# aerius-labs/indexed-merkle-tree-halo2

Measured on AMD Instinct MI355X. Metric: indexed-tree insertions/sec at depth=32 (bn256::Fr), higher is better.
Workload: dtype u32 limbs (9 x 29-bit, Montgomery mod p), 64-bit accumulate

## Files before the change

### indexed-merkle-tree-halo2_amd/csrc/imt_capi.cpp

```cpp
#include "imt_ctx.hpp"
#include "imt_gadget.hpp"
#include <cstring>
#include <new>

using namespace imt;

void* imt_ctx::dev_scratch(size_t slot, size_t bytes) {
    if (slot >= scratch.size()) scratch.resize(slot + 1);
    Scratch& s = scratch[slot];
    if (s.cap >= bytes && s.p) return s.p;
    if (s.p) {
        hipStreamSynchronize(stream);
        hipFree(s.p);
        s.p = nullptr;
        s.cap = 0;
    }
    size_t cap = bytes < 4096 ? 4096 : bytes + bytes / 4;
    hipError_t e = hipMalloc(&s.p, cap);
    if (e != hipSuccess) {
        s.p = nullptr;
        hip_fail(e, "hipMalloc(scratch)");
        return nullptr;
    }
    s.cap = cap;
// ... 105 lines not shown
    IMT_HIP(c, hipStreamSynchronize(c->stream));
    for (auto st : c->side_streams) IMT_HIP(c, hipStreamSynchronize(st));
    for (auto& p : c->prof_pending) {
        float ms = 0;
        if (hipEventElapsedTime(&ms, p.a, p.b) == hipSuccess) {
            c->prof_ms[p.cls] += ms;
            c->prof_n[p.cls] += 1;
        }
        c->prof_pool.push_back(p.a);
        c->prof_pool.push_back(p.b);
    }
    c->prof_pending.clear();
    for (int k = 0; k < IMT_PROF_ALL_CLASSES; k++) {
        if (k < classes) {
            out[2 * k] = c->prof_ms[k];
            out[2 * k + 1] = c->prof_n[k];
        }
        c->prof_ms[k] = c->prof_n[k] = 0;
    }
    return IMT_OK;
}
extern "C" int imt_profile_read(imt_ctx* c, double* out) { return profile_read(c, out, IMT_PROF_CLASSES); }
extern "C" int imt_profile_read_all(imt_ctx* c, double* out) { return profile_read(c, out, IMT_PROF_ALL_CLASSES); }

extern "C" int imt_ctx_set_option(imt_ctx* c, int option, uint64_t value) {
    if (!c) return IMT_ERR_ARG;
    switch (option) {
        case IMT_OPT_COOP_MAX_EVENTS:
            if (value > 0xffffffffu) return c->fail(IMT_ERR_RANGE, "value out of range");
            c->coop_max_events = (uint32_t)value;
            return IMT_OK;
        default:
            return c->fail(IMT_ERR_ARG, "unknown option %d", option);
    }
}

extern "C" const char* imt_version(void) { return "imt-hip gfx950 r4"; }

extern "C" int imt_ctx_create(int device, imt_ctx** out) {
    if (!out) return IMT_ERR_ARG;
    *out = nullptr;
    if (device < 0) return IMT_ERR_NO_DEVICE;
    int count = 0;
    if (hipGetDeviceCount(&count) != hipSuccess || count <= 0 || device >= count) return IMT_ERR_NO_DEVICE;
    imt_ctx* c = new (std::nothrow) imt_ctx();
    if (!c) return IMT_ERR_ALLOC;
    c->device = device;
    std::string err;
    if (!c->hp.init(err)) { delete c; return IMT_ERR_INTERNAL; }
    dev::PoseidonConsts pc;
    c->hp.fill_consts(pc);
    dev::TraceConsts tc;
    c->hp.fill_trace_consts(tc);
    hipError_t e;
    if ((e = hipSetDevice(device)) != hipSuccess || (e = hipStreamCreate(&c->own_stream)) != hipSuccess ||
        (e = launch::upload_consts(pc)) != hipSuccess || (e = launch::upload_trace_consts(tc)) != hipSuccess || (e = hipMalloc((void**)&c->d_err, sizeof(int))) != hipSuccess ||
        (e = hipMalloc((void**)&c->d_zero, (IMT_MAX_DEPTH + 1) * 32)) != hipSuccess) {
        if (c->own_stream) hipStreamDestroy(c->own_stream);
        if (c->d_err) hipFree(c->d_err);
        delete c;
        return e == hipErrorNoDevice ? IMT_ERR_NO_DEVICE : IMT_ERR_HIP;
    }
    c->stream = c->own_stream;
    e = hipMemsetAsync(c->d_err, 0, sizeof(int), c->stream);
    launch::zero_chain(c->stream, c->d_zero, IMT_MAX_DEPTH);
    if (e != hipSuccess || (e = hipStreamSynchronize(c->stream)) != hipSuccess) {
        imt_ctx_destroy(c);
        return IMT_ERR_HIP;
    }
    *out = c;
    return IMT_OK;
}

extern "C" void imt_ctx_destroy(imt_ctx* c) {
    if (!c) return;
    hipSetDevice(c->device);
    hipStreamSynchronize(c->stream);
    for (auto& s : c->scratch)
        if (s.p) hipFree(s.p);
    for (auto& p : c->prof_pending) { hipEventDestroy(p.a); hipEventDestroy(p.b); }
    for (auto& e : c->prof_pool) hipEventDestroy(e);
    if (c->d_err) hipFree(c->d_err);
    if (c->d_zero) hipFree(c->d_zero);
    if (c->own_stream) hipStreamDestroy(c->own_stream);
    delete c;
}

extern "C" const char* imt_last_error(const imt_ctx* c) { return c ? c->last_error.c_str() : "null context"; }

extern "C" int imt_ctx_set_stream(imt_ctx* c, void* s) {
    if (!c) return IMT_ERR_ARG;
    c->stream = s ? (hipStream_t)s : c->own_stream;
    return IMT_OK;
}

extern "C" int imt_ctx_sync(imt_ctx* c) {
    if (!c) return IMT_ERR_ARG;
    int rc = c->set_device();
    if (rc) return rc;
    for (auto st : c->side_streams) IMT_HIP(c, hipStreamSynchronize(st));
    return c->sync_and_check();
}

namespace {

struct Io {
    imt_ctx* c;
    unsigned flags;
    bool dev;
// ... 666 lines not shown
```

### indexed-merkle-tree-halo2_amd/csrc/imt_consts.hpp

```cpp
#pragma once
#include <cstdint>

namespace imt {
namespace dev {

constexpr int NL = 9;
constexpr uint32_t MASK29 = (1u << 29) - 1;

struct Fe {
    uint32_t v[NL];
};

constexpr int RF = 8, RP = 57;
struct PoseidonConsts {
    Fe rc_full[RF][3];
    Fe rc_h2p2[3];
    Fe k_partial[RP];
    Fe mats[2][3][3];
    Fe sp_row[RP][3];
    Fe sp_col[RP][2];
    Fe cap0;
    Fe one;
    Fe from_canon;
    Fe from_mont256;
    Fe to_mont256;
    Fe int_one;
    Fe zero_leaf;
    Fe sc_rc[RF][3];
    Fe sc_mats[RF][3][3];
    Fe rec_k[RP];
    Fe rec_c[RP][4];
    Fe rec_exit[2][3];
    Fe rec_unused[51];
};

struct TraceConsts {
    Fe absorb[3][3];
    Fe full_c[RF][3];
    Fe partial[RP];
    Fe mats[2][3][3];
    Fe row[RP][3];
    Fe col_hat[RP][2];
};
constexpr int TRACE_ROWS_H2 = 1208, TRACE_ROWS_H3 = 1209;

}
}
```

### indexed-merkle-tree-halo2_amd/csrc/imt_kernels.hip

```cpp
#include <algorithm>
#include <hip/hip_runtime.h>
#include <hip/hip_ext.h>

#include "imt_device.hpp"
#include "imt_trace_device.hpp"
#include "imt_launch.hpp"
#include "imt_sweep.hpp"
#if defined(__HIP_DEVICE_COMPILE__)
#include "imt_coop_device.hpp"
#endif

namespace imt {

__constant__ dev::PoseidonConsts g_pc;
__constant__ dev::TraceConsts g_tc;

namespace {
using namespace dev;

#ifndef IMT_BLOCK
#define IMT_BLOCK 256
#endif
#ifndef IMT_HASH_WAVES
#define IMT_HASH_WAVES __attribute__((amdgpu_waves_per_eu(5, 5)))
#endif
#ifndef IMT_COOP_WAVES
#define IMT_COOP_WAVES __attribute__((amdgpu_waves_per_eu(1, 2)))
#endif
constexpr int BLOCK = IMT_BLOCK;

__device__ __forceinline__ size_t gtid() { return (size_t)blockIdx.x * blockDim.x + threadIdx.x; }
__device__ __forceinline__ size_t gtid_again() {
    uint32_t lo = blockIdx.x * blockDim.x + threadIdx.x, hi = (uint32_t)(((uint64_t)blockIdx.x * blockDim.x + threadIdx.x) >> 32);
    asm volatile("" : "+v"(lo), "+v"(hi));
    return ((size_t)hi << 32) | lo;
}
__device__ __forceinline__ void flag_err(int* err, bool ok) {
    if (!ok && err) atomicOr(err, 1);
}

__device__ __forceinline__ void to_int(Fe& r, const Fe& a) {
    mont_mul(r, a, g_pc.int_one);
    canonicalize(r);
}
__device__ __forceinline__ bool int_lt(const Fe& a, const Fe& b) {
    bool lt = false;
#pragma unroll
    for (int i = 0; i < NL; i++) {
        if (a.v[i] != b.v[i]) lt = a.v[i] < b.v[i];
    }
    return lt;
}
__device__ __forceinline__ void fe_from_u64(Fe& r, uint64_t x) {
    Fe t;
#pragma unroll
    for (int i = 0; i < NL; i++) t.v[i] = 0;
    t.v[0] = (uint32_t)x & MASK29;
    t.v[1] = (uint32_t)(x >> 29) & MASK29;
    t.v[2] = (uint32_t)(x >> 58);
    mont_mul(r, t, g_pc.from_canon);
    canonicalize(r);
}

__device__ __forceinline__ void order_pair(Fe& A, Fe& B, bool right, const Fe& cur, const Fe& sv) {
#pragma unroll
    for (int i = 0; i < NL; i++) {
        A.v[i] = right ? sv.v[i] : cur.v[i];
// ... 644 lines not shown
}

struct StoredSibling {
    __device__ __forceinline__ const uint8_t* operator()(const launch::SweepArgs& a, int32_t ss, uint64_t sn) const {
        return ss >= 0 ? a.val_in + (size_t)ss * 32 : (sn < a.len_l ? a.tree_l + sn * 32 : a.zero_l);
    }
};
struct ViewSibling {
    const view::Side& side;
    __device__ __forceinline__ const uint8_t* operator()(const launch::SweepArgs& a, int32_t ss, uint64_t sn) const {
        return replay::sibling_row(side, ss, a.level, sn, a.val_in, a.tree_l, a.len_l, a.zero_l);
    }
};
#if defined(__HIP_DEVICE_COMPILE__)
template <bool TABLES, class Sibling, class Rows = InsertRows>
__device__ __forceinline__ void sweep_body_quad(const launch::SweepArgs& a, Sibling sibling, uint32_t* tab, Rows rows = Rows()) {
    coop::tab_fill(tab, g_pc);
    const size_t t = gtid();
    const size_t q = t >> 2;
    if (q >= a.count) return;
    const unsigned role = (unsigned)t & 3u, ri = role == 3u ? 0u : role;
    const uint32_t x = a.begin + (uint32_t)q;
    const bool leaves = !TABLES && a.mode == launch::SWEEP_LEAVES;
    Fe X, C3, o;
    C3 = g_pc.one;
    if (leaves) {
        flag_err(a.err, leaf_inputs_quad(X, C3, a.pre + (size_t)a.time0[x] * 96, a.fmt_in, ri));
    } else {
        uint32_t k = x, n = 0, e = x;
        const uint8_t* sp = a.zero_l;
        if (TABLES || a.from) {
            k = a.from[x] & ~sweep::LAST_BIT;
            n = a.node_below[x];
            e = a.time_next[x];
            sp = sibling(a, a.sibsrc[x], (uint64_t)(n ^ 1u));
        }
        Fe cur, sv;
        load_packed(cur, a.val_in + (size_t)k * 32);
        load_packed(sv, sp);
        pick_input(X, ri, n & 1u, cur, sv);
        if (role == 0u) {
            if (!TABLES && x == a.last_event && a.node_in) store_packed(a.node_in, cur);
            rows(a, e, sv);
        }
    }
    coop::hash23(tab, o, X, C3, leaves, ri);
    if (role == 1u) {
        store_packed(a.val_out + (size_t)x * 32, o);
        if (!TABLES && x == a.last_event && a.node_out) store_packed(a.node_out, o);
    }
}
#endif
__global__ IMT_HASH_WAVES void __launch_bounds__(BLOCK) k_sweep(launch::SweepArgs a) {
    __shared__ uint32_t stash[NL][BLOCK];
    const size_t t = gtid();
    if (t >= a.count) return;
    const uint32_t x = a.begin + (uint32_t)t;
    Fe A, B, o;
    if (a.mode == launch::SWEEP_LEAVES) {
        const uint8_t* p = a.pre + (size_t)a.time0[x] * 96;
        Fe C;
        bool ok = load_fe(g_pc, A, p, a.fmt_in);
        ok &= load_fe(g_pc, B, p + 32, a.fmt_in);
        ok &= load_fe(g_pc, C, p + 64, a.fmt_in);
#pragma unroll
        for (int i = 0; i < NL; i++) stash[i][threadIdx.x] = C.v[i];
        flag_err(a.err, ok);
    } else {
        uint32_t k = x, n = 0, e = x;
        const uint8_t* sp = a.zero_l;
        if (a.from) {
            k = a.from[x] & ~sweep::LAST_BIT;
            n = a.node_below[x];
            e = a.time_next[x];
            const int32_t ss = a.sibsrc[x];
            const uint64_t sn = (uint64_t)(n ^ 1u);
            sp = ss >= 0 ? a.val_in + (size_t)ss * 32 : (sn < a.len_l ? a.tree_l + sn * 32 : a.zero_l);
        }
        Fe cur, sv;
        load_packed(cur, a.val_in + (size_t)k * 32);
        load_packed(sv, sp);
        if (x == a.last_event && a.node_in) store_packed(a.node_in, cur);
        const bool right = n & 1u;
#pragma unroll
        for (int i = 0; i < NL; i++) {
            A.v[i] = right ? sv.v[i] : cur.v[i];
            B.v[i] = right ? cur.v[i] : sv.v[i];
        }
        uint8_t* row = (e & 1u) ? a.new_sib : a.low_sib;
        if (row) store_fe(g_pc, row + ((uint64_t)a.level * a.lay.level_stride + (uint64_t)(e >> 1) * a.lay.item_stride) * 32, sv, a.fmt_out);
    }
    hash23_stashed(g_pc, o, A, B, a.mode == launch::SWEEP_LEAVES, &stash[0][threadIdx.x], BLOCK);
    store_packed(a.val_out + (size_t)x * 32, o);
    if (x == a.last_event && a.node_out) store_packed(a.node_out, o);
}

__global__ IMT_HASH_WAVES void __launch_bounds__(BLOCK) k_sweep_coop(launch::SweepArgs a) {
#if defined(__HIP_DEVICE_COMPILE__)
    __shared__ uint32_t tab[coop::TAB_DWORDS];
    sweep_body_quad<false>(a, StoredSibling(), tab);
#endif
}

__global__ IMT_HASH_WAVES void __launch_bounds__(BLOCK) k_sweep_mixed(launch::SweepMixedArgs m) {
    const launch::SweepArgs& a = m.sweep;
    const size_t t = gtid();
    if (t >= a.count) return;
    const uint32_t x = a.begin + (uint32_t)t;
    uint32_t k = x, n = 0, e = x;
    const uint8_t* sp = a.zero_l;
    if (a.from) {
        k = a.from[x] & ~sweep::LAST_BIT;
        n = a.node_below[x];
        e = a.time_next[x];
        sp = StoredSibling()(a, a.sibsrc[x], (uint64_t)(n ^ 1u));
    }
    Fe A, B, o, cur, sv;
    load_packed(cur, a.val_in + (size_t)k * 32);
    load_packed(sv, sp);
    if (x == a.last_event && a.node_in) store_packed(a.node_in, cur);
    order_pair(A, B, n & 1u, cur, sv);
    MixedRows{m.erow, m.read_sib}(a, e, sv);
    hash23_stashed(g_pc, o, A, B, false, nullptr, 0);
    store_packed(a.val_out + (size_t)x * 32, o);
    if (x == a.last_event && a.node_out) store_packed(a.node_out, o);
}

__global__ IMT_HASH_WAVES void __launch_bounds__(BLOCK) k_sweep_mixed_coop(launch::SweepMixedArgs m) {
#if defined(__HIP_DEVICE_COMPILE__)
    __shared__ uint32_t tab[coop::TAB_DWORDS];
    sweep_body_quad<false>(m.sweep, StoredSibling(), tab, MixedRows{m.erow, m.read_sib});
#endif
}

__global__ void __launch_bounds__(BLOCK)
k_emit_roots_mixed(const uint8_t* __restrict__ val, uint32_t total, const uint32_t* __restrict__ erow, uint32_t n_ins,
                   uint8_t* __restrict__ old_root, uint8_t* __restrict__ interim_root, uint8_t* __restrict__ new_root,
                   uint8_t* __restrict__ read_root, unsigned fmt_out, uint8_t* __restrict__ node_store) {
    const size_t t = gtid();
    if (t >= total) return;
    const uint32_t e = (uint32_t)t;
    Fe cur;
    load_packed(cur, val + (size_t)e * 32);
    if (e == total - 1 && node_store) store_packed(node_store, cur);
    const uint32_t w = erow[e], kind = w & 3u;
    const size_t i = w >> 2;
    if (kind == 1u) {
// ... 440 lines not shown
        const uint32_t* nodes = reinterpret_cast<const uint32_t*>(j.payload + 128 + (size_t)j.cap * 32);
        const uint64_t node = nodes[i];
        if (node >= j.len_l) return;
        const Word4* s = reinterpret_cast<const Word4*>(j.payload + 128 + i * 32);
        Word4* d = reinterpret_cast<Word4*>(j.tree_l + node * 32);
        d[0] = s[0];
        d[1] = s[1];
        return;
    }
    if (i >= 3) return;
    uint8_t* dst = i == 0 ? j.node_in : (i == 1 ? j.node_out : j.root);
    if (!dst) return;
    const Word4* s = reinterpret_cast<const Word4*>(j.payload + i * 32);
    Word4* d = reinterpret_cast<Word4*>(dst);
    d[0] = s[0];
    d[1] = s[1];
}

__global__ void k_store_top_path(const uint8_t* __restrict__ top_path, uint8_t* __restrict__ tree_nodes,
                                 const uint64_t* __restrict__ tree_off, unsigned l0, unsigned depth) {
    const unsigned l = l0 + threadIdx.x;
    if (l > depth) return;
    const Word4* s = reinterpret_cast<const Word4*>(top_path + (size_t)(l - l0) * 32);
    Word4* d = reinterpret_cast<Word4*>(tree_nodes + tree_off[l] * 32);
    d[0] = s[0];
    d[1] = s[1];
}

__global__ void __launch_bounds__(256) k_mad_peak(uint32_t* out, uint32_t seed, int iters) {
    uint64_t a0 = threadIdx.x + seed, a1 = a0 * 3 + 1, a2 = a0 * 5 + 2, a3 = a0 * 7 + 3;
    uint64_t a4 = a0 * 11 + 4, a5 = a0 * 13 + 5, a6 = a0 * 17 + 6, a7 = a0 * 19 + 7;
    const uint32_t b = (uint32_t)a0 | 1u, c = seed * 77u + 12345u;
    for (int i = 0; i < iters; i++) {
        asm volatile("v_mad_u64_u32 %0, vcc, %8, %9, %0\n v_mad_u64_u32 %1, vcc, %8, %9, %1\n"
                     "v_mad_u64_u32 %2, vcc, %8, %9, %2\n v_mad_u64_u32 %3, vcc, %8, %9, %3\n"
                     "v_mad_u64_u32 %4, vcc, %8, %9, %4\n v_mad_u64_u32 %5, vcc, %8, %9, %5\n"
                     "v_mad_u64_u32 %6, vcc, %8, %9, %6\n v_mad_u64_u32 %7, vcc, %8, %9, %7\n"
                     : "+v"(a0), "+v"(a1), "+v"(a2), "+v"(a3), "+v"(a4), "+v"(a5), "+v"(a6), "+v"(a7)
                     : "v"(b), "v"(c) : "vcc");
    }
    const uint64_t r = a0 ^ a1 ^ a2 ^ a3 ^ a4 ^ a5 ^ a6 ^ a7;
    out[blockIdx.x * blockDim.x + threadIdx.x] = (uint32_t)r ^ (uint32_t)(r >> 32);
}

inline unsigned nblk(size_t n) { return (unsigned)((n + BLOCK - 1) / BLOCK); }

}

namespace launch {

hipError_t upload_consts(const dev::PoseidonConsts& pc) {
    return hipMemcpyToSymbol(HIP_SYMBOL(g_pc), &pc, sizeof(pc), 0, hipMemcpyHostToDevice);
}
hipError_t upload_trace_consts(const dev::TraceConsts& tc) {
    return hipMemcpyToSymbol(HIP_SYMBOL(g_tc), &tc, sizeof(tc), 0, hipMemcpyHostToDevice);
}
void hash_trace_jobs(hipStream_t s, const TraceJobs& a, unsigned fmt_out) {
    size_t most = 0;
    for (int k = 0; k < a.n_jobs; k++) most = std::max(most, a.j[k].n_items);
    if (!most || a.n_jobs <= 0) return;
    auto* k = fmt_out == FMT_MONT256 ? k_hash_trace<FMT_MONT256>
              : fmt_out == FMT_DEVICE ? k_hash_trace<FMT_DEVICE> : k_hash_trace<FMT_CANONICAL>;
    hipLaunchKernelGGL(k, dim3(nblk(most), (unsigned)a.n_jobs), dim3(BLOCK), 0, s, a);
}
void hash_trace(hipStream_t s, const uint8_t* in, size_t n_items, int arity, uint8_t* trace, size_t n_per, size_t row0,
                size_t rows_total, bool item_major, unsigned fmt_in, unsigned fmt_out, int* err) {
    TraceJobs a{};
    a.j[0] = {in, n_items, arity, row0, fmt_in};
    a.n_jobs = 1;
    a.trace = trace; a.n_per = n_per; a.rows_total = rows_total; a.item_major = item_major ? 1 : 0; a.err = err;
    hash_trace_jobs(s, a, fmt_out);
}
void insert_trace_inputs(hipStream_t s, const uint8_t* low_leaf, const uint8_t* new_leaf, const uint64_t* new_index,
                         size_t n, uint8_t* new_low, uint8_t* zero_leaf, unsigned fmt, int* err) {
    if (!n) return;
    hipLaunchKernelGGL(k_insert_trace_inputs, dim3(nblk(n)), dim3(BLOCK), 0, s, low_leaf, new_leaf, new_index, n, new_low,
                       zero_leaf, fmt, err);
}
void path_pairs(hipStream_t s, const PathChains& a, uint32_t coop_max) {
    if (!a.n || a.n_chains <= 0) return;
    if (a.n * 4 * (size_t)a.n_chains <= coop_max)
        hipLaunchKernelGGL(k_path_pairs_coop, dim3(nblk(a.n * 4), (unsigned)a.n_chains), dim3(BLOCK), 0, s, a);
    else
        hipLaunchKernelGGL(k_path_pairs, dim3(nblk(a.n), (unsigned)a.n_chains), dim3(BLOCK), 0, s, a);
}

void hash_batch(hipStream_t s, const uint8_t* in, uint8_t* out, size_t n, int arity, unsigned fmt_in,
                unsigned fmt_out, int* err, uint32_t coop_max) {
    if (!n) return;
    if (n * 4 <= coop_max)
        hipLaunchKernelGGL(k_hash_batch_coop, dim3(nblk(n * 4)), dim3(BLOCK), 0, s, in, out, n, arity, fmt_in, fmt_out, err);
    else
        hipLaunchKernelGGL(k_hash_batch, dim3(nblk(n)), dim3(BLOCK), 0, s, in, out, n, arity, fmt_in, fmt_out, err);
}
void permute_batch(hipStream_t s, const uint8_t* in, uint8_t* out, size_t n, unsigned fmt_in, unsigned fmt_out,
                   int* err) {
    if (!n) return;
    hipLaunchKernelGGL(k_permute_batch, dim3(nblk(n)), dim3(BLOCK), 0, s, in, out, n, fmt_in, fmt_out, err);
}
void convert(hipStream_t s, const uint8_t* in, uint8_t* out, size_t n, unsigned fmt_in, unsigned fmt_out,
             int* err) {
    if (!n) return;
    hipLaunchKernelGGL(k_convert, dim3(nblk(n)), dim3(BLOCK), 0, s, in, out, n, fmt_in, fmt_out, err);
}
void split128(hipStream_t s, const uint8_t* vals, uint8_t* q, uint8_t* r, size_t n, unsigned fmt, int* err) {
    if (!n) return;
// ... 33 lines not shown
                    unsigned fmt_in, unsigned fmt_out, int* err, uint32_t coop_max) {
    (void)fmt_out;
    if (!n) return;
    if (n * 16 <= coop_max)
        hipLaunchKernelGGL(k_insert_chains_coop, dim3(nblk(n * 4), 4), dim3(BLOCK), 0, s, low_leaf, low_index, low_sib,
                           new_leaf, new_index, new_path_index, new_sib, lay, depth, n, trace, fmt_in, err);
    else
        hipLaunchKernelGGL(k_insert_chains, dim3(nblk(n), 4), dim3(BLOCK), 0, s, low_leaf, low_index, low_sib, new_leaf,
                           new_index, new_path_index, new_sib, lay, depth, n, trace, fmt_in, err);
    hipLaunchKernelGGL(k_insert_check, dim3(nblk(n)), dim3(BLOCK), 0, s, old_root, low_leaf, new_root, new_leaf,
                       is_largest, n, trace, fail_out, fmt_in, err);
}
void tree_level(hipStream_t s, const uint8_t* prev, uint8_t* next, size_t n_parents, uint32_t coop_max) {
    if (!n_parents) return;
    if (n_parents * 4 <= coop_max)
        hipLaunchKernelGGL(k_hash_batch_coop, dim3(nblk(n_parents * 4)), dim3(BLOCK), 0, s, prev, next, n_parents, 2,
                           (unsigned)FMT_DEVICE, (unsigned)FMT_DEVICE, (int*)nullptr);
    else
        hipLaunchKernelGGL(k_tree_level, dim3(nblk(n_parents)), dim3(BLOCK), 0, s, prev, next, n_parents);
}
void index_leaves(hipStream_t s, const uint8_t* val, const uint32_t* sorted, uint32_t M, uint64_t base, uint8_t* tree0,
                  int* err) {
    if (!M) return;
    hipLaunchKernelGGL(k_index_leaves, dim3(nblk(M)), dim3(BLOCK), 0, s, val, sorted, M, base, tree0, err);
}
void zero_chain(hipStream_t s, uint8_t* out, unsigned depth) {
    hipLaunchKernelGGL(k_zero_chain, dim3(1), dim3(64), 0, s, out, depth);
}
void extend_root(hipStream_t s, uint8_t* cur, const uint8_t* zero, unsigned from, unsigned to) {
    hipLaunchKernelGGL(k_extend_root, dim3(1), dim3(64), 0, s, cur, zero, from, to);
}
void gather_proof(hipStream_t s, TreeView tv, const uint64_t* index, size_t n, unsigned depth, uint8_t* out,
                  SibLayout lay, unsigned fmt_out) {
    if (!n || !depth) return;
    hipLaunchKernelGGL(k_gather_proof, dim3(nblk(n * depth)), dim3(BLOCK), 0, s, tv, index, n, depth, out, lay,
                       fmt_out);
}
void write_helpers(hipStream_t s, uint64_t index, unsigned depth, uint8_t* out, unsigned fmt_out) {
    if (!depth) return;
    hipLaunchKernelGGL(k_write_helpers, dim3((depth + 63) / 64), dim3(64), 0, s, index, depth, out, fmt_out);
}


void mad_peak(hipStream_t s, uint32_t* out, unsigned blocks, int iters) {
    hipLaunchKernelGGL(k_mad_peak, dim3(blocks), dim3(256), 0, s, out, 1u, iters);
}
void fill_level(hipStream_t s, uint8_t* nodes, size_t n, const uint8_t* zero_l) {
    if (!n) return;
    hipLaunchKernelGGL(k_fill_level, dim3(nblk(n)), dim3(BLOCK), 0, s, nodes, n, zero_l);
}
static void launch_sweep(hipStream_t s, const SweepArgs& a, uint32_t coop_max) {
    if (a.count <= coop_max)
        hipLaunchKernelGGL(k_sweep_coop, dim3(nblk((size_t)a.count * 4)), dim3(BLOCK), 0, s, a);
    else
        hipLaunchKernelGGL(k_sweep, dim3(nblk(a.count)), dim3(BLOCK), 0, s, a);
}
void sweep_leaves(hipStream_t s, const uint8_t* pre, const uint32_t* time0, uint8_t* val0, uint32_t k_begin,
                  uint32_t k_count, unsigned fmt_in, int* err, uint32_t coop_max) {
    if (!k_count) return;
    SweepArgs a{};
    a.mode = SWEEP_LEAVES;
    a.begin = k_begin; a.count = k_count;
    a.pre = pre; a.time0 = time0; a.val_out = val0; a.fmt_in = fmt_in; a.err = err;
    a.last_event = 0xffffffffu;
    launch_sweep(s, a, coop_max);
}
void merge_level(hipStream_t s, sweep::LevelTable in, sweep::LevelOut out, uint32_t total) {
    if (!total) return;
    hipLaunchKernelGGL(k_merge_level, dim3(nblk(total)), dim3(BLOCK), 0, s, in, out, total);
}
static SweepArgs level_args(const uint8_t* val_in, uint8_t* val_out, const uint32_t* from, const int32_t* sibsrc,
                            const uint32_t* node_below, const uint32_t* time_next, const uint8_t* tree_l, uint64_t len_l,
                            const uint8_t* zero_l, uint32_t k_begin, uint32_t k_count, uint8_t* low_sib, uint8_t* new_sib,
                            SibLayout lay, unsigned level, unsigned fmt_out) {
    SweepArgs a{};
    a.mode = SWEEP_LEVEL;
    a.begin = k_begin; a.count = k_count;
    a.val_in = val_in; a.val_out = val_out; a.from = from; a.sibsrc = sibsrc; a.node_below = node_below;
    a.time_next = time_next; a.tree_l = tree_l; a.len_l = len_l; a.zero_l = zero_l; a.level = level;
    a.low_sib = low_sib; a.new_sib = new_sib; a.lay = lay; a.fmt_out = fmt_out;
    a.last_event = 0xffffffffu;
    return a;
}
void sweep_level(hipStream_t s, const uint8_t* val_in, uint8_t* val_out, const uint32_t* from, const int32_t* sibsrc,
                 const uint32_t* node_below, const uint32_t* time_next, const uint8_t* tree_l, uint64_t len_l,
                 const uint8_t* zero_l, uint32_t k_begin, uint32_t k_count, uint8_t* low_sib, uint8_t* new_sib,
                 SibLayout lay, unsigned level, unsigned fmt_out, uint32_t coop_max) {
    if (!k_count) return;
    launch_sweep(s, level_args(val_in, val_out, from, sibsrc, node_below, time_next, tree_l, len_l, zero_l, k_begin, k_count,
                               low_sib, new_sib, lay, level, fmt_out), coop_max);
}
void sweep_upper(hipStream_t s, const uint8_t* val_in, uint8_t* val_out, const uint8_t* zero_l, uint32_t e_begin,
                 uint32_t e_count, uint32_t last_event, uint8_t* node_in, uint8_t* node_out, uint8_t* low_sib,
                 uint8_t* new_sib, SibLayout lay, unsigned level, unsigned fmt_out, uint32_t coop_max) {
    if (!e_count) return;
    SweepArgs a{};
    a.mode = SWEEP_LEVEL;
    a.begin = e_begin; a.count = e_count;
    a.val_in = val_in; a.val_out = val_out; a.zero_l = zero_l; a.level = level;
    a.low_sib = low_sib; a.new_sib = new_sib; a.lay = lay; a.fmt_out = fmt_out;
    a.last_event = last_event; a.node_in = node_in; a.node_out = node_out;
    launch_sweep(s, a, coop_max);
}
static void launch_sweep_mixed(hipStream_t s, const SweepArgs& a, const MixedRoute& r, uint32_t coop_max) {
    const SweepMixedArgs m{a, r.erow, r.read_sib};
    if (a.count <= coop_max)
// ... 203 lines not shown
```

### indexed-merkle-tree-halo2_amd/csrc/imt_launch.hpp

```cpp
#pragma once
#include <hip/hip_runtime_api.h>
#include <cstddef>
#include <cstdint>
#include "imt_consts.hpp"
#include "imt_sweep.hpp"
#include "imt_view.hpp"
#include "imt_replay.hpp"

namespace imt {
namespace launch {

struct SibLayout {
    uint64_t level_stride, item_stride;
};

struct TreeView {
    const uint8_t* nodes;
    const uint64_t* off;
    const uint64_t* len;
    const uint8_t* zero;
    uint64_t index_base = 0;
};

hipError_t upload_consts(const dev::PoseidonConsts& pc);
hipError_t upload_trace_consts(const dev::TraceConsts& tc);

void hash_trace(hipStream_t s, const uint8_t* in, size_t n_items, int arity, uint8_t* trace, size_t n_per, size_t row0,
                size_t rows_total, bool item_major, unsigned fmt_in, unsigned fmt_out, int* err);
struct TraceJobs {
    struct Job {
        const uint8_t* in;
        size_t n_items;
        int arity;
        size_t row0;
        unsigned fmt_in;
    } j[8];
    int n_jobs;
    uint8_t* trace;
    size_t n_per, rows_total;
    int item_major;
    int* err;
};
void hash_trace_jobs(hipStream_t s, const TraceJobs& a, unsigned fmt_out);
void insert_trace_inputs(hipStream_t s, const uint8_t* low_leaf, const uint8_t* new_leaf, const uint64_t* new_index,
                         size_t n, uint8_t* new_low, uint8_t* zero_leaf, unsigned fmt, int* err);
struct PathChains {
    struct Chain {
        const uint8_t* leaf;
        const uint8_t* leaf3;
        const uint64_t* index;
        const uint8_t* sib;
        uint8_t* pairs;
        uint8_t* root_out;
    } c[4];
    int n_chains;
    SibLayout lay;
    unsigned depth;
    size_t n;
    unsigned fmt_in, fmt_out;
    int* err;
};
void path_pairs(hipStream_t s, const PathChains& a, uint32_t coop_max);

void hash_batch(hipStream_t s, const uint8_t* in, uint8_t* out, size_t n, int arity, unsigned fmt_in,
                unsigned fmt_out, int* err, uint32_t coop_max = 0);
void permute_batch(hipStream_t s, const uint8_t* in, uint8_t* out, size_t n, unsigned fmt_in,
                   unsigned fmt_out, int* err);
void convert(hipStream_t s, const uint8_t* in, uint8_t* out, size_t n, unsigned fmt_in,
             unsigned fmt_out, int* err);

void mad_peak(hipStream_t s, uint32_t* out, unsigned blocks, int iters);
void split128(hipStream_t s, const uint8_t* vals, uint8_t* q, uint8_t* r, size_t n, unsigned fmt, int* err);

void path_root(hipStream_t s, const uint8_t* leaf, const uint8_t* leaf3, const uint64_t* index,
               bool is_helper, const uint8_t* sib, SibLayout lay, unsigned depth, size_t n,
               uint8_t* root_out, const uint8_t* expect, unsigned expect_stride, uint8_t* ok_out,
               unsigned fmt_in, unsigned fmt_out, int* err, uint32_t coop_max = 0);
// ... 206 lines not shown
```

### indexed-merkle-tree-halo2_amd/csrc/imt_params.cpp

```cpp
#include "imt_params.hpp"

namespace imt {

namespace {
struct Grain {
    uint8_t b[80];
    int pos = 0;
    int new_bit() {
        int p = pos;
        auto g = [&](int k) { return b[(p + k) % 80]; };
        int nb = g(62) ^ g(51) ^ g(38) ^ g(23) ^ g(13) ^ g(0);
        b[p] = (uint8_t)nb;
        pos = (p + 1) % 80;
        return nb;
    }
    int next() {
        while (!new_bit()) new_bit();
        return new_bit();
    }
    void take254(uint8_t le[32]) {
        std::memset(le, 0, 32);
        for (int i = 253; i >= 0; i--)
            if (next()) le[i / 8] |= (uint8_t)(1u << (i % 8));
    }
// ... 2 lines not shown

void HostPoseidon::permute_plain(HFr s[3]) const {
    for (int r = 0; r < 65; r++) {
        for (int i = 0; i < 3; i++) s[i] = F.add(s[i], rc[r][i]);
        const int nsb = (r < 4 || r >= 61) ? 3 : 1;
        for (int i = 0; i < nsb; i++) {
            HFr x2 = F.mul(s[i], s[i]), x4 = F.mul(x2, x2);
            s[i] = F.mul(x4, s[i]);
        }
        HFr n[3];
        for (int i = 0; i < 3; i++) {
            n[i] = F.mul(mds[i][0], s[0]);
            n[i] = F.add(n[i], F.mul(mds[i][1], s[1]));
            n[i] = F.add(n[i], F.mul(mds[i][2], s[2]));
        }
        s[0] = n[0]; s[1] = n[1]; s[2] = n[2];
    }
}

void HostPoseidon::permute_opt(HFr s[3]) const {
    auto sbox = [&](HFr& x) {
        HFr x2 = F.mul(x, x), x4 = F.mul(x2, x2);
        x = F.mul(x4, x);
    };
    auto dense = [&](const HFr m[3][3]) {
        HFr n[3];
        for (int i = 0; i < 3; i++) {
            n[i] = F.mul(m[i][0], s[0]);
            n[i] = F.add(n[i], F.mul(m[i][1], s[1]));
            n[i] = F.add(n[i], F.mul(m[i][2], s[2]));
        }
        s[0] = n[0]; s[1] = n[1]; s[2] = n[2];
    };
    for (int r = 0; r < 65; r++) {
        if (r < 4 || r >= 61) {
            const int fr = r < 4 ? r : r - 57;
            for (int i = 0; i < 3; i++) s[i] = F.add(s[i], rc_full[fr][i]);
            for (int i = 0; i < 3; i++) sbox(s[i]);
            dense(r == 3 ? pre : mds);
        } else {
            const int p = r - 4;
            HFr y = F.add(s[0], k_partial[p]);
            sbox(y);
            HFr n0 = F.mul(sp_row[p][0], y);
            n0 = F.add(n0, F.mul(sp_row[p][1], s[1]));
            n0 = F.add(n0, F.mul(sp_row[p][2], s[2]));
            s[1] = F.add(s[1], F.mul(sp_col[p][0], y));
            s[2] = F.add(s[2], F.mul(sp_col[p][1], y));
            s[0] = n0;
        }
    }
}

void HostPoseidon::permute_rec(HFr s[3]) const {
    auto sbox = [&](HFr& x) {
        HFr x2 = F.mul(x, x), x4 = F.mul(x2, x2);
        x = F.mul(x4, x);
    };
    auto dot = [&](const HFr* c, const HFr* v, int n) {
        HFr o = F.zero();
        for (int i = 0; i < n; i++) o = F.add(o, F.mul(c[i], v[i]));
        return o;
    };
    auto full = [&](int f) {
        for (int i = 0; i < 3; i++) s[i] = F.add(s[i], sc_rc[f][i]);
        for (int i = 0; i < 3; i++) sbox(s[i]);
        const HFr n0 = (f == 0 || f == 4) ? dot(sc_mats[f][0], s, 3) : F.add(F.add(s[0], s[1]), s[2]);
        const HFr n1 = dot(sc_mats[f][1], s, 3), n2 = dot(sc_mats[f][2], s, 3);
        s[0] = n0; s[1] = n1; s[2] = n2;
    };
    for (int f = 0; f < 4; f++) full(f);
    HFr a = s[0], b = s[1], z3 = F.zero(), z2 = s[2];
    for (int r = 0; r < 57; r++) {
        HFr z = F.add(a, rec_k[r]);
        sbox(z);
        HFr w;
        if (r == 0) {
            w = F.add(b, z);
        } else if (r == 1) {
            const HFr v2[2] = {a, z2};
            w = F.add(dot(rec_c[1], v2, 2), F.add(z3, z));
        } else {
            const HFr v4[4] = {a, b, z3, z2};
            w = F.add(dot(rec_c[r], v4, 4), z);
        }
        b = a; a = w; z3 = z2; z2 = z;
    }
    const HFr v3[3] = {a, b, z3};
    s[0] = a;
    s[1] = F.add(dot(rec_exit[0], v3, 3), z2);
    s[2] = F.add(dot(rec_exit[1], v3, 3), z2);
    for (int f = 4; f < 8; f++) full(f);
}

void HostPoseidon::permute_spec(HFr s[3]) const {
    auto x5c = [&](HFr& x, const HFr& c) {
        HFr x2 = F.mul(x, x), x4 = F.mul(x2, x2);
        x = F.add(F.mul(x4, x), c);
    };
    auto dense = [&](const HFr m[3][3]) {
        HFr n[3];
        for (int i = 0; i < 3; i++) {
            n[i] = F.mul(m[i][0], s[0]);
            n[i] = F.add(n[i], F.mul(m[i][1], s[1]));
            n[i] = F.add(n[i], F.mul(m[i][2], s[2]));
        }
        s[0] = n[0]; s[1] = n[1]; s[2] = n[2];
    };
    for (int i = 0; i < 3; i++) s[i] = F.add(s[i], tr_start[0][i]);
    for (int r = 1; r <= 4; r++) {
        for (int i = 0; i < 3; i++) x5c(s[i], tr_start[r][i]);
        dense(r == 4 ? tr_pre : mds);
    }
    for (int p = 0; p < 57; p++) {
        x5c(s[0], tr_partial[p]);
        HFr n0 = F.mul(tr_row[p][0], s[0]);
        n0 = F.add(n0, F.mul(tr_row[p][1], s[1]));
        n0 = F.add(n0, F.mul(tr_row[p][2], s[2]));
        s[1] = F.add(F.mul(tr_col_hat[p][0], s[0]), s[1]);
        s[2] = F.add(F.mul(tr_col_hat[p][1], s[0]), s[2]);
        s[0] = n0;
    }
    for (int r = 0; r < 4; r++) {
        for (int i = 0; i < 3; i++) x5c(s[i], r < 3 ? tr_end[r][i] : F.zero());
        dense(mds);
    }
}

HFr HostPoseidon::hash2(const HFr& a, const HFr& b) const {
    HFr s[3] = {cap0, a, b};
    permute_opt(s);
    s[1] = F.add(s[1], F.one());
    permute_opt(s);
    return s[1];
}
HFr HostPoseidon::hash3(const HFr& a, const HFr& b, const HFr& c) const {
    HFr s[3] = {cap0, a, b};
    permute_opt(s);
    s[1] = F.add(s[1], c);
    s[2] = F.add(s[2], F.one());
    permute_opt(s);
    return s[1];
}

bool HostPoseidon::init(std::string& err) {
    Grain g;
    int n = 0;
    auto put = [&](int width, unsigned v) {
        for (int i = width - 1; i >= 0; i--) g.b[n++] = (v >> i) & 1;
    };
    put(2, 1); put(4, 0); put(12, 254); put(12, 3); put(10, 8); put(10, 57); put(30, 0x3fffffffu);
    for (int i = 0; i < 160; i++) g.new_bit();
    uint8_t le[32];
    for (int r = 0; r < 65; r++)
        for (int i = 0; i < 3; i++) {
            do { g.take254(le); } while (!F.from_bytes(rc[r][i], le));
        }
    HFr xs[3], ys[3];
    auto norej = [&](HFr& o) {
        g.take254(le);
        uint64_t v[4];
        std::memcpy(v, le, 32);
        if (HField::geq_p(v)) HField::sub_p(v);
        std::memcpy(le, v, 32);
        F.from_bytes(o, le);
    };
    for (auto& x : xs) norej(x);
    for (auto& y : ys) norej(y);
    for (int i = 0; i < 3; i++)
        for (int j = 0; j < 3; j++) mds[i][j] = F.inverse(F.add(xs[i], ys[j]));
    HFr two32 = F.from_u64(1ULL << 32);
    cap0 = F.mul(two32, two32);

    auto matvec = [&](const HFr m[3][3], const HFr v[3], HFr o[3]) {
        for (int i = 0; i < 3; i++) {
            o[i] = F.mul(m[i][0], v[0]);
            o[i] = F.add(o[i], F.mul(m[i][1], v[1]));
            o[i] = F.add(o[i], F.mul(m[i][2], v[2]));
        }
    };
    for (int r = 0; r < 4; r++)
        for (int i = 0; i < 3; i++) rc_full[r][i] = rc[r][i];
    HFr w[3] = {F.zero(), F.zero(), F.zero()};
    for (int p = 4; p <= 60; p++) {
        HFr v[3], mw[3];
        matvec(mds, w, mw);
        for (int i = 0; i < 3; i++) v[i] = F.add(mw[i], rc[p][i]);
        k_partial[p - 4] = v[0];
        w[0] = F.zero(); w[1] = v[1]; w[2] = v[2];
    }
    {
        HFr mw[3];
        matvec(mds, w, mw);
        for (int i = 0; i < 3; i++) rc_full[4][i] = F.add(rc[61][i], mw[i]);
// ... 172 lines not shown
        };
        HFr minv[3][3];
        {
            auto cof = [&](int r0, int r1, int c0, int c1) {
                return F.sub(F.mul(mds[r0][c0], mds[r1][c1]), F.mul(mds[r0][c1], mds[r1][c0]));
            };
            HFr adj[3][3];
            for (int i = 0; i < 3; i++)
                for (int j = 0; j < 3; j++) {
                    const int r0 = (j + 1) % 3, r1 = (j + 2) % 3, c0 = (i + 1) % 3, c1 = (i + 2) % 3;
                    adj[i][j] = cof(r0, r1, c0, c1);
                }
            HFr det = F.add(F.add(F.mul(mds[0][0], adj[0][0]), F.mul(mds[0][1], adj[1][0])), F.mul(mds[0][2], adj[2][0]));
            if (F.is_zero(det)) { err = "singular MDS"; return false; }
            HFr di = F.inverse(det);
            for (int i = 0; i < 3; i++)
                for (int j = 0; j < 3; j++) minv[i][j] = F.mul(adj[i][j], di);
        }
        for (int i = 0; i < 3; i++) tr_start[0][i] = rc[0][i];
        for (int r = 1; r < 4; r++) matvec(minv, rc[r], tr_start[r]);
        HFr acc[3] = {rc[61][0], rc[61][1], rc[61][2]};
        for (int p = 56; p >= 0; p--) {
            HFr tmp[3];
            matvec(minv, acc, tmp);
            tr_partial[p] = tmp[0];
            acc[0] = rc[4 + p][0];
            acc[1] = F.add(tmp[1], rc[4 + p][1]);
            acc[2] = F.add(tmp[2], rc[4 + p][2]);
        }
        matvec(minv, acc, tr_start[4]);
        for (int r = 0; r < 3; r++) matvec(minv, rc[62 + r], tr_end[r]);
        HFr mt[3][3], a[3][3];
        for (int i = 0; i < 3; i++)
            for (int j = 0; j < 3; j++) mt[i][j] = a[i][j] = mds[j][i];
        for (int k = 0; k < 57; k++) {
            const int p = 56 - k;
            HFr det = F.sub(F.mul(a[1][1], a[2][2]), F.mul(a[1][2], a[2][1]));
            if (F.is_zero(det)) { err = "singular MDS minor"; return false; }
            HFr di = F.inverse(det);
            HFr hi[2][2] = {{F.mul(a[2][2], di), F.mul(F.sub(F.zero(), a[1][2]), di)},
                            {F.mul(F.sub(F.zero(), a[2][1]), di), F.mul(a[1][1], di)}};
            tr_row[p][0] = a[0][0];
            tr_row[p][1] = F.add(F.mul(hi[0][0], a[1][0]), F.mul(hi[0][1], a[2][0]));
            tr_row[p][2] = F.add(F.mul(hi[1][0], a[1][0]), F.mul(hi[1][1], a[2][0]));
            tr_col_hat[p][0] = a[0][1];
            tr_col_hat[p][1] = a[0][2];
            HFr prime[3][3] = {{F.one(), F.zero(), F.zero()}, {F.zero(), a[1][1], a[1][2]}, {F.zero(), a[2][1], a[2][2]}};
            mat_mul(mt, prime, a);
        }
        for (int i = 0; i < 3; i++)
            for (int j = 0; j < 3; j++) tr_pre[i][j] = a[j][i];
    }

    for (uint64_t t = 0; t < 6; t++) {
        HFr a[3] = {F.from_u64(t * 7919), F.from_u64(t * t + 1), F.mul(cap0, F.from_u64(t + 3))};
        if (t == 4) a[0] = a[1] = a[2] = F.sub(F.zero(), F.one());
        if (t == 5) a[0] = a[1] = a[2] = F.mul(cap0, cap0);
        HFr b[3] = {a[0], a[1], a[2]}, sc[3] = {a[0], a[1], a[2]}, c3[3] = {a[0], a[1], a[2]};
        permute_plain(a);
        permute_opt(b);
        permute_rec(sc);
        if (!(a[0] == b[0] && a[1] == b[1] && a[2] == b[2])) {
            err = "optimised Poseidon schedule disagrees with the plain form";
            return false;
        }
        if (!(a[0] == sc[0] && a[1] == sc[1] && a[2] == sc[2])) {
            err = "device (recurrence) Poseidon schedule disagrees with the plain form";
            return false;
        }
        permute_spec(c3);
        if (!(a[0] == c3[0] && a[1] == c3[1] && a[2] == c3[2])) {
            err = "halo2-base form of the Poseidon schedule disagrees with the plain form";
            return false;
        }
    }
    return true;
}

void HostPoseidon::fill_trace_consts(dev::TraceConsts& tc) const {
    for (int i = 0; i < 3; i++) {
        tc.absorb[0][i] = to_dev(tr_start[0][i]);
        tc.absorb[1][i] = to_dev(i == 2 ? F.add(tr_start[0][i], F.one()) : tr_start[0][i]);
        tc.absorb[2][i] = to_dev(i == 1 ? F.add(tr_start[0][i], F.one()) : tr_start[0][i]);
    }
    for (int f = 0; f < 8; f++)
        for (int i = 0; i < 3; i++)
            tc.full_c[f][i] = to_dev(f < 4 ? tr_start[f + 1][i] : f < 7 ? tr_end[f - 4][i] : F.zero());
    for (int p = 0; p < 57; p++) {
        tc.partial[p] = to_dev(tr_partial[p]);
        for (int i = 0; i < 3; i++) tc.row[p][i] = to_dev(tr_row[p][i]);
        for (int i = 0; i < 2; i++) tc.col_hat[p][i] = to_dev(tr_col_hat[p][i]);
    }
    for (int i = 0; i < 3; i++)
        for (int j = 0; j < 3; j++) {
            tc.mats[0][i][j] = to_dev(mds[i][j]);
            tc.mats[1][i][j] = to_dev(tr_pre[i][j]);
        }
}

dev::Fe HostPoseidon::int_to_dev_limbs(const uint8_t le[32]) const {
    dev::Fe o;
    for (int i = 0; i < dev::NL; i++) {
        uint32_t v = 0;
        for (int k = 0; k < 29; k++) {
            int bit = 29 * i + k;
            if (bit < 256 && ((le[bit / 8] >> (bit % 8)) & 1)) v |= 1u << k;
        }
        o.v[i] = v;
    }
    return o;
}

dev::Fe HostPoseidon::to_dev(const HFr& x) const {
    HFr two29 = F.from_u64(1ULL << 29);
    HFr t = x;
    for (int i = 0; i < 9; i++) t = F.mul(t, two29);
    uint8_t le[32];
    F.to_bytes(le, t);
    return int_to_dev_limbs(le);
}

void HostPoseidon::fill_consts(dev::PoseidonConsts& pc) const {
    for (int r = 0; r < 8; r++)
        for (int i = 0; i < 3; i++) pc.rc_full[r][i] = to_dev(rc_full[r][i]);
    pc.rc_h2p2[0] = to_dev(rc_full[0][0]);
    pc.rc_h2p2[1] = to_dev(F.add(rc_full[0][1], F.one()));
    pc.rc_h2p2[2] = to_dev(rc_full[0][2]);
    for (int p = 0; p < 57; p++) {
        pc.k_partial[p] = to_dev(k_partial[p]);
// ... 36 lines not shown
```

### indexed-merkle-tree-halo2_amd/csrc/imt_params.hpp

```cpp
#pragma once
#include "imt_consts.hpp"
#include "imt_fr_host.hpp"
#include <string>
#include <vector>

namespace imt {

struct HostPoseidon {
    HField F;
    HFr rc[65][3];
    HFr mds[3][3];
    HFr rc_full[8][3];
    HFr k_partial[57];
    HFr pre[3][3];
    HFr sp_row[57][3];
    HFr sp_col[57][2];
    HFr cap0;
    HFr sc_rc[8][3];
    HFr sc_mats[8][3][3];
    HFr rec_k[57], rec_c[57][4], rec_exit[2][3];
    HFr tr_start[5][3], tr_partial[57], tr_end[3][3];
    HFr tr_pre[3][3];
    HFr tr_row[57][3], tr_col_hat[57][2];

    bool init(std::string& err);

    void permute_plain(HFr s[3]) const;
    void permute_opt(HFr s[3]) const;
    void permute_rec(HFr s[3]) const;
    void permute_spec(HFr s[3]) const;
    void fill_trace_consts(dev::TraceConsts& tc) const;
    HFr hash2(const HFr& a, const HFr& b) const;
    HFr hash3(const HFr& a, const HFr& b, const HFr& c) const;

    dev::Fe to_dev(const HFr& x) const;
    dev::Fe int_to_dev_limbs(const uint8_t le[32]) const;
    void fill_consts(dev::PoseidonConsts& pc) const;
};

}
```

Measured before the change: 3.651 million.

## Precompute Poseidon first-round S-boxes for capacity and zero siblings in sweep hash

After: 3.679 million (median of 6 runs). About the same (+0.8%).

```diff
diff --git a/indexed-merkle-tree-halo2_amd/csrc/imt_capi.cpp b/indexed-merkle-tree-halo2_amd/csrc/imt_capi.cpp
--- a/indexed-merkle-tree-halo2_amd/csrc/imt_capi.cpp
+++ b/indexed-merkle-tree-halo2_amd/csrc/imt_capi.cpp
@@ -181,9 +181,12 @@
     c->hp.fill_consts(pc);
     dev::TraceConsts tc;
     c->hp.fill_trace_consts(tc);
+    dev::SweepConsts sw;
+    c->hp.fill_sweep_consts(sw);
     hipError_t e;
     if ((e = hipSetDevice(device)) != hipSuccess || (e = hipStreamCreate(&c->own_stream)) != hipSuccess ||
-        (e = launch::upload_consts(pc)) != hipSuccess || (e = launch::upload_trace_consts(tc)) != hipSuccess || (e = hipMalloc((void**)&c->d_err, sizeof(int))) != hipSuccess ||
+        (e = launch::upload_consts(pc)) != hipSuccess || (e = launch::upload_sweep_consts(sw)) != hipSuccess ||
+        (e = launch::upload_trace_consts(tc)) != hipSuccess || (e = hipMalloc((void**)&c->d_err, sizeof(int))) != hipSuccess ||
         (e = hipMalloc((void**)&c->d_zero, (IMT_MAX_DEPTH + 1) * 32)) != hipSuccess) {
         if (c->own_stream) hipStreamDestroy(c->own_stream);
         if (c->d_err) hipFree(c->d_err);
diff --git a/indexed-merkle-tree-halo2_amd/csrc/imt_consts.hpp b/indexed-merkle-tree-halo2_amd/csrc/imt_consts.hpp
--- a/indexed-merkle-tree-halo2_amd/csrc/imt_consts.hpp
+++ b/indexed-merkle-tree-halo2_amd/csrc/imt_consts.hpp
@@ -34,6 +34,12 @@
     Fe rec_unused[51];
 };
 
+constexpr int SWEEP_ZERO_LEVELS = 64;
+struct SweepConsts {
+    Fe cap5;
+    Fe zero5[SWEEP_ZERO_LEVELS];
+};
+
 struct TraceConsts {
     Fe absorb[3][3];
     Fe full_c[RF][3];
diff --git a/indexed-merkle-tree-halo2_amd/csrc/imt_kernels.hip b/indexed-merkle-tree-halo2_amd/csrc/imt_kernels.hip
--- a/indexed-merkle-tree-halo2_amd/csrc/imt_kernels.hip
+++ b/indexed-merkle-tree-halo2_amd/csrc/imt_kernels.hip
@@ -6,6 +6,7 @@
 #include "imt_trace_device.hpp"
 #include "imt_launch.hpp"
 #include "imt_sweep.hpp"
+#include "imt_sweep_hash.hpp"
 #if defined(__HIP_DEVICE_COMPILE__)
 #include "imt_coop_device.hpp"
 #endif
@@ -13,6 +14,7 @@
 namespace imt {
 
 __constant__ dev::PoseidonConsts g_pc;
+__constant__ dev::SweepConsts g_sw;
 __constant__ dev::TraceConsts g_tc;
 
 namespace {
@@ -763,31 +765,21 @@
 }
 #endif
 __global__ IMT_HASH_WAVES void __launch_bounds__(BLOCK) k_sweep(launch::SweepArgs a) {
-    __shared__ uint32_t stash[NL][BLOCK];
     const size_t t = gtid();
     if (t >= a.count) return;
     const uint32_t x = a.begin + (uint32_t)t;
     Fe A, B, o;
-    if (a.mode == launch::SWEEP_LEAVES) {
-        const uint8_t* p = a.pre + (size_t)a.time0[x] * 96;
-        Fe C;
-        bool ok = load_fe(g_pc, A, p, a.fmt_in);
-        ok &= load_fe(g_pc, B, p + 32, a.fmt_in);
-        ok &= load_fe(g_pc, C, p + 64, a.fmt_in);
-#pragma unroll
-        for (int i = 0; i < NL; i++) stash[i][threadIdx.x] = C.v[i];
-        flag_err(a.err, ok);
-    } else {
-        uint32_t k = x, n = 0, e = x;
-        const uint8_t* sp = a.zero_l;
-        if (a.from) {
-            k = a.from[x] & ~sweep::LAST_BIT;
-            n = a.node_below[x];
-            e = a.time_next[x];
-            const int32_t ss = a.sibsrc[x];
-            const uint64_t sn = (uint64_t)(n ^ 1u);
-            sp = ss >= 0 ? a.val_in + (size_t)ss * 32 : (sn < a.len_l ? a.tree_l + sn * 32 : a.zero_l);
-        }
+    uint32_t k = x, n = 0, e = x;
+    const uint8_t* sp = a.zero_l;
+    if (a.from) {
+        k = a.from[x] & ~sweep::LAST_BIT;
+        n = a.node_below[x];
+        e = a.time_next[x];
+        const int32_t ss = a.sibsrc[x];
+        const uint64_t sn = (uint64_t)(n ^ 1u);
+        sp = ss >= 0 ? a.val_in + (size_t)ss * 32 : (sn < a.len_l ? a.tree_l + sn * 32 : a.zero_l);
+    }
+    {
         Fe cur, sv;
         load_packed(cur, a.val_in + (size_t)k * 32);
         load_packed(sv, sp);
@@ -801,9 +793,27 @@
         uint8_t* row = (e & 1u) ? a.new_sib : a.low_sib;
         if (row) store_fe(g_pc, row + ((uint64_t)a.level * a.lay.level_stride + (uint64_t)(e >> 1) * a.lay.item_stride) * 32, sv, a.fmt_out);
     }
-    hash23_stashed(g_pc, o, A, B, a.mode == launch::SWEEP_LEAVES, &stash[0][threadIdx.x], BLOCK);
+    const Fe* zero5 = (!a.from && a.level < (unsigned)SWEEP_ZERO_LEVELS) ? &g_sw.zero5[a.level] : nullptr;
+    hash2_sweep(g_pc, g_sw, o, A, B, zero5);
     store_packed(a.val_out + (size_t)x * 32, o);
     if (x == a.last_event && a.node_out) store_packed(a.node_out, o);
+}
+
+__global__ IMT_HASH_WAVES void __launch_bounds__(BLOCK) k_sweep_leaves(launch::SweepArgs a) {
+    __shared__ uint32_t stash[NL][BLOCK];
+    const size_t t = gtid();
+    if (t >= a.count) return;
+    const uint32_t x = a.begin + (uint32_t)t;
+    const uint8_t* p = a.pre + (size_t)a.time0[x] * 96;
+    Fe A, B, C, o;
+    bool ok = load_fe(g_pc, A, p, a.fmt_in);
+    ok &= load_fe(g_pc, B, p + 32, a.fmt_in);
+    ok &= load_fe(g_pc, C, p + 64, a.fmt_in);
+#pragma unroll
+    for (int i = 0; i < NL; i++) stash[i][threadIdx.x] = C.v[i];
+    flag_err(a.err, ok);
+    hash23_stashed(g_pc, o, A, B, true, &stash[0][threadIdx.x], BLOCK);
+    store_packed(a.val_out + (size_t)x * 32, o);
 }
 
 __global__ IMT_HASH_WAVES void __launch_bounds__(BLOCK) k_sweep_coop(launch::SweepArgs a) {
@@ -1350,6 +1360,9 @@
 hipError_t upload_consts(const dev::PoseidonConsts& pc) {
     return hipMemcpyToSymbol(HIP_SYMBOL(g_pc), &pc, sizeof(pc), 0, hipMemcpyHostToDevice);
 }
+hipError_t upload_sweep_consts(const dev::SweepConsts& sw) {
+    return hipMemcpyToSymbol(HIP_SYMBOL(g_sw), &sw, sizeof(sw), 0, hipMemcpyHostToDevice);
+}
 hipError_t upload_trace_consts(const dev::TraceConsts& tc) {
     return hipMemcpyToSymbol(HIP_SYMBOL(g_tc), &tc, sizeof(tc), 0, hipMemcpyHostToDevice);
 }
@@ -1489,6 +1502,8 @@
 static void launch_sweep(hipStream_t s, const SweepArgs& a, uint32_t coop_max) {
     if (a.count <= coop_max)
         hipLaunchKernelGGL(k_sweep_coop, dim3(nblk((size_t)a.count * 4)), dim3(BLOCK), 0, s, a);
+    else if (a.mode == SWEEP_LEAVES)
+        hipLaunchKernelGGL(k_sweep_leaves, dim3(nblk(a.count)), dim3(BLOCK), 0, s, a);
     else
         hipLaunchKernelGGL(k_sweep, dim3(nblk(a.count)), dim3(BLOCK), 0, s, a);
 }
diff --git a/indexed-merkle-tree-halo2_amd/csrc/imt_launch.hpp b/indexed-merkle-tree-halo2_amd/csrc/imt_launch.hpp
--- a/indexed-merkle-tree-halo2_amd/csrc/imt_launch.hpp
+++ b/indexed-merkle-tree-halo2_amd/csrc/imt_launch.hpp
@@ -23,6 +23,7 @@
 };
 
 hipError_t upload_consts(const dev::PoseidonConsts& pc);
+hipError_t upload_sweep_consts(const dev::SweepConsts& sw);
 hipError_t upload_trace_consts(const dev::TraceConsts& tc);
 
 void hash_trace(hipStream_t s, const uint8_t* in, size_t n_items, int arity, uint8_t* trace, size_t n_per, size_t row0,
diff --git a/indexed-merkle-tree-halo2_amd/csrc/imt_params.cpp b/indexed-merkle-tree-halo2_amd/csrc/imt_params.cpp
--- a/indexed-merkle-tree-halo2_amd/csrc/imt_params.cpp
+++ b/indexed-merkle-tree-halo2_amd/csrc/imt_params.cpp
@@ -78,7 +78,9 @@
     }
 }
 
-void HostPoseidon::permute_rec(HFr s[3]) const {
+void HostPoseidon::permute_rec(HFr s[3]) const { permute_sweep(s, nullptr, nullptr, false); }
+
+void HostPoseidon::permute_sweep(HFr s[3], const HFr* lane0_5, const HFr* lane2_5, bool row1_only) const {
     auto sbox = [&](HFr& x) {
         HFr x2 = F.mul(x, x), x4 = F.mul(x2, x2);
         x = F.mul(x4, x);
@@ -91,6 +93,12 @@
     auto full = [&](int f) {
         for (int i = 0; i < 3; i++) s[i] = F.add(s[i], sc_rc[f][i]);
         for (int i = 0; i < 3; i++) sbox(s[i]);
+        if (f == 0 && lane0_5) s[0] = *lane0_5;
+        if (f == 0 && lane2_5) s[2] = *lane2_5;
+        if (f == 7 && row1_only) {
+            s[1] = dot(sc_mats[f][1], s, 3);
+            return;
+        }
         const HFr n0 = (f == 0 || f == 4) ? dot(sc_mats[f][0], s, 3) : F.add(F.add(s[0], s[1]), s[2]);
         const HFr n1 = dot(sc_mats[f][1], s, 3), n2 = dot(sc_mats[f][2], s, 3);
         s[0] = n0; s[1] = n1; s[2] = n2;
@@ -166,6 +174,14 @@
     s[1] = F.add(s[1], c);
     s[2] = F.add(s[2], F.one());
     permute_opt(s);
+    return s[1];
+}
+
+HFr HostPoseidon::hash2_sweep(const HFr& a, const HFr& b, int zero_level) const {
+    HFr s[3] = {cap0, a, b};
+    permute_sweep(s, &sw_cap5, zero_level >= 0 ? &sw_zero5[zero_level] : nullptr, false);
+    s[1] = F.add(s[1], F.one());
+    permute_sweep(s, nullptr, nullptr, true);
     return s[1];
 }
 
@@ -444,6 +460,20 @@
             for (int j = 0; j < 3; j++) tr_pre[i][j] = a[j][i];
     }
 
+    {
+        auto pow5 = [&](const HFr& x) {
+            const HFr x2 = F.mul(x, x);
+            return F.mul(F.mul(x2, x2), x);
+        };
+        sw_cap5 = pow5(F.add(cap0, rc[0][0]));
+        HFr z = hash3(F.zero(), F.zero(), F.zero());
+        for (int l = 0; l < dev::SWEEP_ZERO_LEVELS; l++) {
+            sw_zero[l] = z;
+            sw_zero5[l] = pow5(F.add(z, rc[0][2]));
+            z = hash2(z, z);
+        }
+    }
+
     for (uint64_t t = 0; t < 6; t++) {
         HFr a[3] = {F.from_u64(t * 7919), F.from_u64(t * t + 1), F.mul(cap0, F.from_u64(t + 3))};
         if (t == 4) a[0] = a[1] = a[2] = F.sub(F.zero(), F.one());
@@ -466,7 +496,28 @@
             return false;
         }
     }
+    const int heights[5] = {0, 1, 31, 32, dev::SWEEP_ZERO_LEVELS - 1};
+    for (int t = 0; t < 6 + 5; t++) {
+        const int zl = t < 6 ? -1 : heights[t - 6];
+        HFr a = F.mul(cap0, F.from_u64(7919u * (uint64_t)t + 5)), b = F.from_u64((uint64_t)t * t + 1);
+        if (t == 1) a = b = F.zero();
+        if (t == 2) a = b = F.sub(F.zero(), F.one());
+        if (zl >= 0) b = sw_zero[zl];
+        HFr s[3] = {cap0, a, b};
+        permute_plain(s);
+        s[1] = F.add(s[1], F.one());
+        permute_plain(s);
+        if (!(s[1] == hash2_sweep(a, b, zl))) {
+            err = "level hash of the batch insertion disagrees with the plain form";
+            return false;
+        }
+    }
     return true;
+}
+
+void HostPoseidon::fill_sweep_consts(dev::SweepConsts& sw) const {
+    sw.cap5 = to_dev(sw_cap5);
+    for (int l = 0; l < dev::SWEEP_ZERO_LEVELS; l++) sw.zero5[l] = to_dev(sw_zero5[l]);
 }
 
 void HostPoseidon::fill_trace_consts(dev::TraceConsts& tc) const {
diff --git a/indexed-merkle-tree-halo2_amd/csrc/imt_params.hpp b/indexed-merkle-tree-halo2_amd/csrc/imt_params.hpp
--- a/indexed-merkle-tree-halo2_amd/csrc/imt_params.hpp
+++ b/indexed-merkle-tree-halo2_amd/csrc/imt_params.hpp
@@ -19,6 +19,7 @@
     HFr sc_rc[8][3];
     HFr sc_mats[8][3][3];
     HFr rec_k[57], rec_c[57][4], rec_exit[2][3];
+    HFr sw_cap5, sw_zero5[dev::SWEEP_ZERO_LEVELS], sw_zero[dev::SWEEP_ZERO_LEVELS];
     HFr tr_start[5][3], tr_partial[57], tr_end[3][3];
     HFr tr_pre[3][3];
     HFr tr_row[57][3], tr_col_hat[57][2];
@@ -28,6 +29,9 @@
     void permute_plain(HFr s[3]) const;
     void permute_opt(HFr s[3]) const;
     void permute_rec(HFr s[3]) const;
+    void permute_sweep(HFr s[3], const HFr* lane0_5, const HFr* lane2_5, bool row1_only) const;
+    HFr hash2_sweep(const HFr& a, const HFr& b, int zero_level) const;
+    void fill_sweep_consts(dev::SweepConsts& sw) const;
     void permute_spec(HFr s[3]) const;
     void fill_trace_consts(dev::TraceConsts& tc) const;
     HFr hash2(const HFr& a, const HFr& b) const;
diff --git a/indexed-merkle-tree-halo2_amd/csrc/imt_sweep_hash.hpp b/indexed-merkle-tree-halo2_amd/csrc/imt_sweep_hash.hpp
--- /dev/null
+++ b/indexed-merkle-tree-halo2_amd/csrc/imt_sweep_hash.hpp
@@ -0,0 +1,91 @@
+#pragma once
+#include "imt_device.hpp"
+
+namespace imt {
+namespace dev {
+
+IMT_HD void permute_sweep(const PoseidonConsts& pc, const SweepConsts& sw, Fe s[3], bool second, const Fe* zero5) {
+    constexpr int NSTEP = RF + RP;
+    Fe z3;
+#pragma unroll
+    for (int i = 0; i < NL; i++) z3.v[i] = 0;
+#pragma unroll 1
+    for (int st = 0; st < NSTEP; st++) {
+        if (st < RF / 2 || st >= RF / 2 + RP) {
+            const int fr = st < RF / 2 ? st : st - RP;
+            if (fr == RF / 2) {
+                const Fe v[3] = {s[0], s[1], z3};
+                const Fe zl = s[2];
+#pragma unroll 1
+                for (int i = 0; i < 2; i++) {
+                    Fe n;
+                    mont_dot_uc<3, false>(n, pc.rec_exit[i], v, v[0]);
+                    add_lazy(n, n, zl);
+                    normalize(n);
+                    s[1] = s[2]; s[2] = n;
+                }
+            }
+            const bool head = st == 0 && !second, tail = st == NSTEP - 1 && second;
+            const Fe* rc = (st == 0) ? (second ? pc.rc_h2p2 : pc.rc_full[0]) : pc.sc_rc[fr];
+            if (head) {
+                s[0] = sw.cap5;
+            } else {
+                add_lazy(s[0], s[0], rc[0]);
+                sbox(s[0]);
+            }
+            add_lazy(s[1], s[1], rc[1]);
+            sbox(s[1]);
+            if (head && zero5) {
+                s[2] = *zero5;
+            } else {
+                add_lazy(s[2], s[2], rc[2]);
+                sbox(s[2]);
+            }
+            const Fe(*mat)[3] = pc.sc_mats[fr];
+            Fe n1;
+            mont_dot_uc<3, false>(n1, mat[1], s, s[0]);
+            if (!tail) {
+                Fe n0, n2;
+                if (fr == 0 || fr == RF / 2) {
+                    mont_dot_uc<3, false>(n0, mat[0], s, s[0]);
+                } else {
+                    add_lazy(n0, s[0], s[1]);
+                    add_lazy(n0, n0, s[2]);
+                    normalize(n0);
+                }
+                mont_dot_uc<3, false>(n2, mat[2], s, s[0]);
+                s[0] = n0; s[2] = n2;
+            }
+            s[1] = n1;
+        } else {
+            const int r = st - RF / 2;
+            Fe z, w;
+            add_lazy(z, s[0], pc.rec_k[r]);
+            sbox(z);
+            if (r >= 2) {
+                const Fe v[4] = {s[0], s[1], z3, s[2]};
+                mont_dot_uc<4, true>(w, pc.rec_c[r], v, z);
+            } else if (r == 1) {
+                const Fe v[2] = {s[0], s[2]};
+                Fe e;
+                add_lazy(e, z3, z);
+                mont_dot_uc<2, true, false>(w, pc.rec_c[1], v, e);
+            } else {
+                add_lazy(w, s[1], z);
+                normalize(w);
+            }
+            s[1] = s[0]; s[0] = w; z3 = s[2]; s[2] = z;
+        }
+    }
+}
+
+IMT_HD void hash2_sweep(const PoseidonConsts& pc, const SweepConsts& sw, Fe& out, const Fe& a, const Fe& b, const Fe* zero5) {
+    Fe s[3] = {a, a, b};
+#pragma unroll 1
+    for (int blk = 0; blk < 2; blk++) permute_sweep(pc, sw, s, blk == 1, zero5);
+    out = s[1];
+    canonicalize(out);
+}
+
+}
+}
```
